# theteamatx/x-edr-trajectory-planning

Measured on AMD Instinct MI355X. Metric: time-optimal path timings/s (7-DOF, 2000 s-samples), 1/2/4/8 MI355X + %HBM roofline, higher is better.
Workload: dtype f64

## Files before the change

### x-edr-trajectory-planning_amd/csrc/tpamd_sweep_inst.hip

```cpp
#include "tpamd_launch.h"
#include "tpamd_sweep_joint.h"

#if !defined(TPAMD_INST_D) || !defined(TPAMD_INST_E)
#error "compile with -DTPAMD_INST_D=<joints> -DTPAMD_INST_E=<0|2>"
#endif

namespace tpamd {

template <>
void launch_sweep_joint<TPAMD_INST_D, TPAMD_INST_E>(int B, hipStream_t st, int N, int max_loops,
                                                    const JointSource &src, const Workspace &ws,
                                                    const tpamd_path_outputs *out) {
  hipLaunchKernelGGL((k_sweep_joint<TPAMD_INST_D, TPAMD_INST_E>), dim3(B), dim3(128),
                     (sweep_joint_lds_bytes<TPAMD_INST_D, TPAMD_INST_E>(N)), st, N, max_loops, src, ws,
                     out->time, out->s, out->sd, out->sdd, out->last_extremal_index,
                     out->max_time_increment, out->status, out->qd, out->qdd);
}

template <>
hipError_t configure_sweep_joint<TPAMD_INST_D, TPAMD_INST_E>() {
  return hipFuncSetAttribute(reinterpret_cast<const void *>(&k_sweep_joint<TPAMD_INST_D, TPAMD_INST_E>),
                             hipFuncAttributeMaxDynamicSharedMemorySize, 160 * 1024);
}

template <>
hipError_t sweep_joint_attributes<TPAMD_INST_D, TPAMD_INST_E>(hipFuncAttributes *attr) {
  return hipFuncGetAttributes(attr, reinterpret_cast<const void *>(&k_sweep_joint<TPAMD_INST_D, TPAMD_INST_E>));
}

}
```

### x-edr-trajectory-planning_amd/csrc/tpamd_sweep_joint.h

```cpp
#pragma once

#include <type_traits>

#include "tpamd_kernels.h"

namespace tpamd {

__device__ __forceinline__ double uniform_f64(double v) {
  const int lo = __builtin_amdgcn_readfirstlane(__double2loint(v));
  const int hi = __builtin_amdgcn_readfirstlane(__double2hiint(v));
  return __hiloint2double(hi, lo);
}
__device__ __forceinline__ double readlane_f64(double v, int lane) {
  const int lo = __builtin_amdgcn_readlane(__double2loint(v), lane);
  const int hi = __builtin_amdgcn_readlane(__double2hiint(v), lane);
  return __hiloint2double(hi, lo);
}
__device__ __forceinline__ int uniform_i32(int v) { return __builtin_amdgcn_readfirstlane(v); }
__device__ __forceinline__ int lds_word(const int *p) {
  return *(const volatile __attribute__((address_space(3))) int *)p;
}

template <int CTRL>
__device__ __forceinline__ double dpp_f64(double v) {
// ... 1160 lines not shown
        const bool iso_k = iso_at(at_l, N, k), iso_km1 = iso_at(at_l, N, k - 1),
                   iso_km2 = iso_at(at_l, N, k - 2);
        const bool l_mod = iso_k || iso_km2;
        const double m_l = l_mod ? z0[k - 1] : m0[k - 1];
        const double fsmax_l = l_mod ? Xz[k - 1] : X0[k - 1];
        const double m_c = iso_km1 ? z0[k] : m0[k];
        const double X_c = iso_km1 ? Xz[k] : X0[k];
        const double Y_c = iso_km1 ? Xz[k] : Y0[k];
        const double m_r = iso_k ? z0[k + 1] : m0[k + 1];
        const double Y_r = iso_k ? Xz[k + 1] : Y0[k + 1];
        const double fsmin_r = iso_k ? Yz[k + 1] : Y0[k + 1];
        const double sd2p = (m_r - m_c) / ds;
        const double sd2p_min = 2 * Y_c;
        const double sd2p_max = 2 * X_c;
        const bool sink_or_source = (sd2p < sd2p_min) || (sd2p > sd2p_max);
        const bool skipped_sdd = (X_c > 0) && (Y_r < 0);
        const bool skipped_sd2 = (m_c > m_l - kTiny) && (m_c > m_r - kTiny);
        if ((skipped_sd2 || skipped_sdd) && sink_or_source) {
          const double fw = m_l + 2.0 * ds * fsmax_l;
          const double bw = m_r - 2.0 * ds * fsmin_r;
          double mn = z0[k];
          if (fw < mn) mn = fw;
          if (bw < mn) mn = bw;
          ws.fix_val[pb + k] = (0.0 < mn) ? mn : 0.0;
          flag = 1;
        }
      }
      ff_l[k] = flag;
    };
    auto drain_detect = [&]() {
      JointSweep<D, E>::wave_lds_sync();
      for (int e0 = 0; e0 < nslow; e0 += 64)
        if (e0 + lane < nslow) detect_one(slow[e0 + lane]);
      nslow = 0;
      JointSweep<D, E>::wave_lds_sync();
    };
    double m0c[UF], X0c[UF], Y0c[UF];
    auto load_segment = [&](int cb) {
#pragma unroll
      for (int u = 0; u < UF; u++) {
        const int c = cb + 2 * u + w;
        const int k = 62 * c + lane - 1;
        const int kc = (c >= 1 && 62 * c + 62 < N) ? k : cl(k);
        m0c[u] = m0[kc]; X0c[u] = X0[kc]; Y0c[u] = Y0[kc];
      }
    };
    const bool owner = (lane >= 1) && (lane <= 62);
    for (int seg = 0; seg < nsg; seg++) {
    const int cb = seg * kSegChunks;
    load_segment(cb);
    unsigned listed = 0u;
#pragma unroll
    for (int u = 0; u < UF; u++) {
      const int k = 62 * (cb + 2 * u + w) + lane - 1;
      const bool inside = owner && (k >= 1) && (k <= N - 2);
      const int kb = max(k, 2);
      const bool near_iso = (iso_l[kb] | iso_l[kb - 1] | iso_l[kb - 2]) != 0;
      const double m_c = m0c[u], X_c = X0c[u], Y_c = Y0c[u];
      const double m0l = dpp_f64<0x138>(m_c);
      const double m0r = dpp_f64<0x130>(m_c), Y0r = dpp_f64<0x130>(Y_c);
      const double sd2p = (m0r - m_c) / ds;
      const double sd2p_min = 2 * Y_c;
      const double sd2p_max = 2 * X_c;
      const bool sink_or_source = (sd2p < sd2p_min) || (sd2p > sd2p_max);
      const bool skipped_sdd = (X_c > 0) && (Y0r < 0);
      const bool skipped_sd2 = (m_c > m0l - kTiny) && (m_c > m0r - kTiny);
      const bool fix = (skipped_sd2 || skipped_sdd) && sink_or_source;
      const bool to_list = inside && (near_iso || fix);
      if (owner && k >= 0 && k < N && !to_list) ff_l[k] = 0;
      listed |= (unsigned)to_list << u;
    }
    list_samples(listed, cb);
    drain_detect();
    }
    __threadfence_block();
    __syncthreads();
    TPAMD_ACCC(21, tp0);

    auto final_one = [&](int j, double &m, double &X, double &Y, double &m_next) -> bool {
      bool refit = false;
      m = 0.0; X = 0.0; Y = 0.0; m_next = 0.0;
      const bool f_next = (j + 1 <= N - 2) && ff_l[j + 1];
      const bool f_self = ff_l[j];
      const bool f_prev = (j >= 1) && ff_l[j - 1];
      const bool iso_p = iso_at(at_l, N, j - 1), iso_n = iso_at(at_l, N, j + 1);
      if (f_next || (!f_self && f_prev)) {
        m = z0[j];
        if (iso_p || iso_n) { X = Xz[j]; Y = Yz[j]; }
        else refit = true;
      } else if (f_self) {
        m = fv[j];
        refit = true;
      } else if (iso_n) {
        m = z0[j]; X = Xz[j]; Y = Yz[j];
      } else if (iso_p) {
        m = z0[j]; X = Xz[j]; Y = Xz[j];
      } else {
        m = m0[j]; X = X0[j]; Y = Y0[j];
      }
      const int jn = j + 1;
      if (jn <= N - 1) {
        if (jn + 1 <= N - 2 && ff_l[jn + 1]) m_next = z0[jn];
        else if (ff_l[jn]) m_next = fv[jn];
        else if (ff_l[jn - 1]) m_next = z0[jn];
        else if (iso_at(at_l, N, jn + 1) || iso_at(at_l, N, jn - 1)) m_next = z0[jn];
        else m_next = m0[jn];
      }
      return refit;
    };
    auto drain_final = [&]() {
      JointSweep<D, E>::wave_lds_sync();
      for (int e0 = 0; e0 < nslow; e0 += 64) {
        const bool valid = e0 + lane < nslow;
        double m = 0.0, X = 0.0, Y = 0.0, m_next = 0.0;
        bool refit = false;
        int j = 0;
        if (valid) {
          j = slow[e0 + lane];
          refit = final_one(j, m, X, Y, m_next);
          if (!refit) P.finalize(j, m, X, Y, m_next);
        }
        if (P.count + 64 > kRefitCap) P.template flush<true>(diag);
        P.append(refit, j, m, m_next);
      }
      nslow = 0;
      JointSweep<D, E>::wave_lds_sync();
    };
    for (int seg = 0; seg < nsg; seg++) {
    const int cb = seg * kSegChunks;
    if (!kOne) load_segment(cb);
    unsigned listed = 0u;
#pragma unroll
    for (int u = 0; u < UF; u++) {
      const int j = 62 * (cb + 2 * u + w) + lane - 1;
      const bool mine = owner && (j >= 0) && (j < N);
      const int jb = max(j, 1);
      const bool busy = (ff_l[jb - 1] | ff_l[jb] | ff_l[jb + 1] | ff_l[jb + 2] |
                         iso_l[jb - 1] | iso_l[jb] | iso_l[jb + 1] | iso_l[jb + 2]) != 0;
      const double m0r = dpp_f64<0x130>(m0c[u]);
      if (mine && !busy) P.finalize(j, m0c[u], X0c[u], Y0c[u], (j + 1 <= N - 1) ? m0r : 0.0);
      listed |= (unsigned)(mine && busy) << u;
    }
    list_samples(listed, cb);
    drain_final();
    }
    P.template flush<true>(diag);
    __threadfence_block();
    __syncthreads();
    TPAMD_ACCC(22, tp0);
    };
    if (nseg == 1) fast_form(std::true_type{});
    else fast_form(std::false_type{});
    return;
  }

  for (int base = 64 * w; base < N; base += 128) {
    const int j = base + lane;
    const bool need = (j < N) & ((iso_l[cl(j - 1)] | iso_l[cl(j + 1)]) != 0);
    if (P.count + 64 > kRefitCap) P.template flush<false>(diag);
    P.append(need, j, need ? z0[j] : 0.0, 0.0);
  }
  P.template flush<false>(diag);
  __threadfence_block();
  __syncthreads();
  TPAMD_ACCC(20, tp0);

  for (int k0 = tid; k0 < N; k0 += 128 * U) {
    double m0l[U], m0c[U], m0r[U], z0l[U], z0c[U], z0r[U], X0l[U], X0c[U], Y0c[U], Y0r[U];
    double Xzl[U], Xzc[U], Xzr[U], Yzr[U];
#pragma unroll
    for (int u = 0; u < U; u++) {
      const int k = k0 + 128 * u;
      const int kl = cl(k - 1), kc = cl(k), kr = cl(k + 1);
      m0l[u] = m0[kl]; m0c[u] = m0[kc]; m0r[u] = m0[kr];
      X0l[u] = X0[kl]; X0c[u] = X0[kc];
      Y0c[u] = Y0[kc]; Y0r[u] = Y0[kr];
      const bool ik = iso_at(at_l, N, k), ik1 = iso_at(at_l, N, k - 1), ik2 = iso_at(at_l, N, k - 2);
      z0l[u] = (ik || ik2) ? z0[kl] : 0.0;
      z0c[u] = ik1 ? z0[kc] : 0.0;
      z0r[u] = ik ? z0[kr] : 0.0;
      Xzl[u] = (ik || ik2) ? Xz[kl] : 0.0;
      Xzc[u] = ik1 ? Xz[kc] : 0.0;
      Xzr[u] = ik ? Xz[kr] : 0.0;
      Yzr[u] = ik ? Yz[kr] : 0.0;
    }
#pragma unroll
    for (int u = 0; u < U; u++) {
      const int k = k0 + 128 * u;
      if (k >= N) continue;
      uint8_t flag = 0;
      if (k >= 1 && k <= N - 2) {
        const bool iso_k = iso_at(at_l, N, k), iso_km1 = iso_at(at_l, N, k - 1),
                   iso_km2 = iso_at(at_l, N, k - 2);
        const bool l_mod = iso_k || iso_km2;
        const double m_l = l_mod ? z0l[u] : m0l[u];
        const double fsmax_l = l_mod ? Xzl[u] : X0l[u];
        const double m_c = iso_km1 ? z0c[u] : m0c[u];
        const double X_c = iso_km1 ? Xzc[u] : X0c[u];
        const double Y_c = iso_km1 ? Xzc[u] : Y0c[u];
        const double m_r = iso_k ? z0r[u] : m0r[u];
        const double Y_r = iso_k ? Xzr[u] : Y0r[u];
        const double fsmin_r = iso_k ? Yzr[u] : Y0r[u];
        const double sd2p = (m_r - m_c) / ds;
        const double sd2p_min = 2 * Y_c;
        const double sd2p_max = 2 * X_c;
        const bool sink_or_source = (sd2p < sd2p_min) || (sd2p > sd2p_max);
        const bool skipped_sdd = (X_c > 0) && (Y_r < 0);
        const bool skipped_sd2 = (m_c > m_l - kTiny) && (m_c > m_r - kTiny);
        if ((skipped_sd2 || skipped_sdd) && sink_or_source) {
          const double fw = m_l + 2.0 * ds * fsmax_l;
          const double bw = m_r - 2.0 * ds * fsmin_r;
          double mn = z0[k];
          if (fw < mn) mn = fw;
          if (bw < mn) mn = bw;
          ws.fix_val[pb + k] = (0.0 < mn) ? mn : 0.0;
          flag = 1;
        }
      }
      ff_l[k] = flag;
    }
  }
  __threadfence_block();
  __syncthreads();
  TPAMD_ACCC(21, tp0);

  for (int base = 256 * w; base < N; base += 512) {
    double m0c[U], z0c[U], X0c[U], Y0c[U], Xzc[U], Yzc[U], fvc[U], m0n[U], z0n[U], fvn[U];
#pragma unroll
    for (int u = 0; u < U; u++) {
      const int j = base + 64 * u + lane;
      const int jc = cl(j), jn = cl(j + 1);
      m0c[u] = m0[jc]; z0c[u] = z0[jc]; X0c[u] = X0[jc]; Y0c[u] = Y0[jc];
      m0n[u] = m0[jn]; z0n[u] = z0[jn];
      const bool near_iso = iso_at(at_l, N, jc - 1) || iso_at(at_l, N, jc + 1);
      Xzc[u] = near_iso ? Xz[jc] : 0.0;
      Yzc[u] = near_iso ? Yz[jc] : 0.0;
      fvc[u] = ff_l[jc] ? fv[jc] : 0.0;
      fvn[u] = ff_l[jn] ? fv[jn] : 0.0;
    }
#pragma unroll
    for (int u = 0; u < U; u++) {
      const int j = base + 64 * u + lane;
      const bool active = j < N;
      double m = 0.0, X = 0.0, Y = 0.0, m_next = 0.0;
      bool refit = false;
      if (active) {
        const bool f_next = (j + 1 <= N - 2) && ff_l[j + 1];
        const bool f_self = ff_l[j];
        const bool f_prev = (j >= 1) && ff_l[j - 1];
        const bool iso_p = iso_at(at_l, N, j - 1), iso_n = iso_at(at_l, N, j + 1);
        if (f_next || (!f_self && f_prev)) {
          m = z0c[u];
          if (iso_p || iso_n) { X = Xzc[u]; Y = Yzc[u]; }
          else refit = true;
        } else if (f_self) {
          m = fvc[u];
          refit = true;
        } else if (iso_n) {
          m = z0c[u]; X = Xzc[u]; Y = Yzc[u];
        } else if (iso_p) {
          m = z0c[u]; X = Xzc[u]; Y = Xzc[u];
        } else {
          m = m0c[u]; X = X0c[u]; Y = Y0c[u];
        }
        const int jn = j + 1;
        if (jn <= N - 1) {
          if (jn + 1 <= N - 2 && ff_l[jn + 1]) m_next = z0n[u];
          else if (ff_l[jn]) m_next = fvn[u];
          else if (ff_l[jn - 1]) m_next = z0n[u];
          else if (iso_at(at_l, N, jn + 1) || iso_at(at_l, N, jn - 1)) m_next = z0n[u];
          else m_next = m0n[u];
        }
        if (!refit) P.finalize(j, m, X, Y, m_next);
      }
      if (P.count + 64 > kRefitCap) P.template flush<true>(diag);
      P.append(refit, j, m, m_next);
    }
  }
  P.template flush<true>(diag);
  __threadfence_block();
  __syncthreads();
  TPAMD_ACCC(22, tp0);
}

template <int D, int E = 0>
struct SweepLds {
  static constexpr int R = 2 * D + E + 2;
  static constexpr int kRingDoubles = 2 * 2 * TileCfg<D>::kSamples * R;
  __host__ __device__ static constexpr int n2(int N) { return (N + 1) & ~1; }
  __host__ __device__ static constexpr int words(int N) { return ((N + 31) / 32 + 1) & ~1; }
  __host__ __device__ static constexpr int type_bytes(int N) { return ((N + 15) / 16) * 16; }
  __host__ __device__ static constexpr size_t bytes(int N) {
    return (size_t)n2(N) * 8 + (size_t)kRingDoubles * 8 + type_bytes(N) + 64 +
           2 * (size_t)words(N) * 4 + 16 * 8 + 32;
  }
};
template <int D, int E = 0>
__host__ __device__ inline size_t sweep_joint_lds_bytes(int N) {
  return SweepLds<D, E>::bytes(N);
}

constexpr int kSweepWavesPerEu = 2;
constexpr int kSweepWavesPerEuWide = 1;
template <int D, int E = 0>
__global__ void __launch_bounds__(128)
__attribute__((amdgpu_waves_per_eu((D > 8) ? kSweepWavesPerEuWide : kSweepWavesPerEu,
                                   (D > 8) ? kSweepWavesPerEuWide : kSweepWavesPerEu)))
k_sweep_joint(int stride, int max_loops, JointSource src, Workspace ws, double *t_out, double *s_out,
              double *sd_out, double *sdd_out, int32_t *lei_out, double *dtmax_out,
              int32_t *status_out, double *qd_out, double *qdd_out) {
  extern __shared__ double lds[];
  typedef JointSweep<D, E> JS;
  typedef SweepLds<D, E> LL;
  const int b = uniform_i32(path_of_block(ws, blockIdx.x));
  const int lane = threadIdx.x & 63;
  const int N = path_samples(ws, b, stride);
  const int w = uniform_i32((int)(threadIdx.x >> 6));
  const int tid = threadIdx.x;
  const size_t pb = (size_t)b * stride;
  const uint32_t bits = ws.err_bits[b];
  if (bits & kErrSkip) return;
  if (bits) {
    if (tid == 0) {
      status_out[b] = status_from_bits(bits);
      if (lei_out) lei_out[b] = 0;
      if (dtmax_out) dtmax_out[b] = -1.0;
    }
    return;
  }
  JS S;
  S.N = N; S.lane = lane;
  S.ds = ws.ds[b];
  S.two_ds = 2.0 * S.ds;
  S.sd2 = lds;
  double *ring = lds + LL::n2(N);
  S.tiles = ring + (size_t)w * 2 * JS::kTile * JS::R;
  uint8_t *typel = reinterpret_cast<uint8_t *>(ring + LL::kRingDoubles);
  S.typel = typel;
  int *xchg = reinterpret_cast<int *>(typel + LL::type_bytes(N));
  const int nw = LL::words(N);
  uint32_t *dirty = reinterpret_cast<uint32_t *>(xchg + 16);
  uint32_t *zero = dirty + nw;
  double *aml = reinterpret_cast<double *>(zero + nw);
  double *red = aml + 16;
  S.dirty = dirty;
  S.aml = aml;
  S.sdd_g = sdd_out + pb;
  S.m_g = ws.m + pb;
  S.rec = src.q12 + pb * JS::R;
  S.qd_g = qd_out ? qd_out + pb * D : nullptr;
  S.qdd_g = qdd_out ? qdd_out + pb * D : nullptr;
  S.end_idx = 0;
  S.tag0 = -1; S.tag1 = -1;
  double *sd2 = S.sd2;
  const double sd_start = ws.sd_start[b];
#ifdef TPAMD_DIAG
  long long(&diag)[32] = S.diag;
  long long(&diagx)[kDiagExt] = S.diagx;
  for (int k = 0; k < 32; k++) diag[k] = 0;
  for (int k = 0; k < kDiagExt; k++) diagx[k] = 0;
  volatile long long *fw_stamp = reinterpret_cast<volatile long long *>(red + 2);
#define TPAMD_DIAG_PTR S.diag
#else
#define TPAMD_DIAG_PTR nullptr
#endif
  boundary_passes_for_path<D, E>(src, ws, b, N, stride, tid, reinterpret_cast<uint8_t *>(sd2),
                           reinterpret_cast<uint8_t *>(sd2) + LL::type_bytes(N),
                           reinterpret_cast<char *>(ring), typel, (ws.keep_boundary & 1) != 0,
                           TPAMD_DIAG_PTR);
  constexpr int C = 2 * D + E;
  const double *lim_lo = src.lim + (size_t)b * 2 * C, *lim_hi = lim_lo + C;
  {
    typedef JointLayout<D> L;
    const double kInf = __longlong_as_double(0x7ff0000000000000LL);
    const bool is_cand = lane < L::kCandLanes;
    const int c = is_cand ? lane / L::PARTS : 0;
    const int p = lane % L::PARTS;
    const int r = c >> 1;
    S.own_off = r;
    S.lim = is_cand ? ((c & 1) ? lim_hi[r] : lim_lo[r]) : qnan();
#pragma unroll
    for (int k = 0; k < L::RPL; k++) {
      int j = p + k * L::PARTS;
      if (j >= D) j = (p < D) ? p : 0;
      S.chk_off[k] = j;
      S.chk_hi[k] = lim_hi[j];
    }
    const bool is_vel = lane < D;
    S.vel_off = is_vel ? lane : 0;
    S.vel_hi = is_vel ? lim_hi[D + lane] : kInf;
    S.vel_lo = is_vel ? 0.0 : -kInf;
    S.vel_mode = 0;
    if (E > 0) {
      if (lane >= D && lane < D + E) {
        S.vel_off = D;
        S.vel_mode = 1 + (lane - D);
        S.vel_hi = lim_hi[2 * D + (lane - D)];
        S.vel_lo = lim_lo[2 * D + (lane - D)];
      }
#pragma unroll
      for (int k = 0; k < (E ? E : 1); k++) S.ex_hi[k] = lim_hi[2 * D + k];
    }
  }
  S.row_lo = (lane < C) ? lim_lo[lane] : 0.0;
  S.row_hi = (lane < C) ? lim_hi[lane] : 0.0;
  {
    typedef JointLayout<D> L;
    const double kInf = __longlong_as_double(0x7ff0000000000000LL);
    const int p = lane & (L::GRP - 1);
#pragma unroll
    for (int i = 0; i < L::CPL; i++) {
      const int cand = p + L::GRP * i;
      const bool has = cand < 2 * D;
      const int row = has ? (cand >> 1) : 0;
      S.v_off[i] = row;
      S.v_lim[i] = has ? ((cand & 1) ? lim_hi[row] : lim_lo[row]) : qnan();
    }
#pragma unroll
    for (int i = 0; i < L::VPL; i++) {
      const int row = p + L::GRP * i;
      const bool has = row < D;
      S.vv_off[i] = has ? row : 0;
      S.vv_hi[i] = has ? lim_hi[D + row] : kInf;
      S.va_hi[i] = has ? lim_hi[row] : kInf;
    }
  }

  for (int i = tid; i < N; i += 128) {
    sd2[i] = qnan();
    S.sdd_g[i] = qnan();
  }
  for (int i = tid; i < 2 * nw; i += 128) dirty[i] = 0u;
  if (tid < D) aml[tid] = ws.amax ? ws.amax[(size_t)b * D + tid] : 0.0;
  __syncthreads();
  if (tid == 0) {
    xchg[2] = 0;
    xchg[6] = 0;
    sd2[0] = sd_start * sd_start;
    sd2[N - 1] = 0;
  }
  __syncthreads();

  int status = 0;
  int iforw_lo = 0, iback_hi = N - 1, iback_lo, iforw_hi, icrit, icrit_lo, icrit_hi;
  typename JS::Prefetch pf;
  pf.tag = -1;
  TPAMD_T0C(t_all);
  int emitted_hi = 0, upper_lo = N;
  bool first_pair_in_order = false;
  if (w == 0) {
    const int r = S.template add_extremal<false>(iback_hi, pf);
    if (lane == 0) { xchg[0] = r; xchg[7] = S.end_idx; }
  } else {
    const int r = S.template add_extremal<true>(iforw_lo, pf);
    if (lane == 0) { xchg[1] = r; xchg[8] = S.end_idx; }
  }
  __threadfence_block();
  __syncthreads();
  const int end_b = uniform_i32(xchg[7]), end_f = uniform_i32(xchg[8]);
  if (!(end_f + 70 < end_b)) {
    first_pair_in_order = true;
    for (int i = tid; i < N; i += 128) {
      sd2[i] = qnan();
      S.sdd_g[i] = qnan();
    }
    __syncthreads();
    if (tid == 0) {
      sd2[0] = sd_start * sd_start;
      sd2[N - 1] = 0;
    }
    __threadfence_block();
    __syncthreads();
  }
  if (first_pair_in_order) {
    if (w == 0) {
      const int r = S.template add_extremal<false>(iback_hi, pf);
      if (lane == 0) xchg[0] = r;
    }
    __threadfence_block();
    __syncthreads();
    if (w == 1) {
      const int r = S.template add_extremal<true>(iforw_lo, pf);
      if (lane == 0) xchg[1] = r;
    } else {
      upper_lo = min(S.end_idx + 3, N);
      S.emit_range(upper_lo, N - 1, 0, 1);
    }
    __threadfence_block();
    __syncthreads();
  }
  iback_lo = uniform_i32(xchg[0]);
  iforw_hi = uniform_i32(xchg[1]);
  TPAMD_ACCC(9, t_all);
  icrit_hi = iback_lo;
  if ((iforw_hi < icrit_hi) && ((icrit_hi < N - 2) && (icrit_hi >= 2))) {
    if (w == 0) S.put_sd2(icrit_hi, qnan());
    icrit_hi++;
    iback_lo++;
  }
  icrit_lo = iforw_hi;
  const int zlast = uniform_i32(S.last_flagged_below(icrit_hi));
  const double *m_g = ws.m + pb;
  if (max_loops <= 0) max_loops = max(100, 10 * N);
  double *crit_m = reinterpret_cast<double *>(xchg + 10);
  auto post_next_critical_point = [&](int lo) {
    TPAMD_T0(t0);
    int ic = uniform_i32(S.next_critical_point(lo, icrit_hi, zlast));
    TPAMD_ACC(2, t0);
#if defined(TPAMD_DIAG) && !defined(TPAMD_DIAG_LIGHT)
    {
      TPAMD_T0(tl_);
      if (ic != S.next_critical_point_literal(lo, icrit_hi)) TPAMD_CNT(7);
      TPAMD_ACC(18, tl_);
    }
#endif
    if (ic < 0 || ic >= N) ic = (int)(0.5 * (lo + icrit_hi));
    const double mc = m_g[min(max(ic, 0), N - 1)], mp = m_g[min(max(ic - 1, 0), N - 1)];
    if (ic >= 1) {
      const int ts = ic / JS::kTile;
      const int tag = (ts & 1) ? S.tag1 : S.tag0;
      if (tag != ts && pf.tag != ts) S.issue_tile_loads(ts, pf);
    }
    if (lane == 0) {
      xchg[9] = ic;
      crit_m[0] = mc;
      crit_m[1] = mp;
    }
  };
  __syncthreads();
  if (w == 1 && iforw_hi < icrit_hi) post_next_critical_point(icrit_lo);
  __threadfence_block();
  __syncthreads();
  for (int loop = 0; loop < max_loops; loop++) {
    if (iforw_hi >= icrit_hi) break;
    TPAMD_CNT(11);
#ifdef TPAMD_DIAG
    int bw_case = 2;
    long long bw_left = 0;
#endif
    icrit = uniform_i32(xchg[9]);
    const double m_c = uniform_f64(crit_m[0]), m_p = uniform_f64(crit_m[1]);
    if (w == 0 && icrit >= 1) {
      const int ts = (icrit - 1) / JS::kTile;
      const int tag = (ts & 1) ? S.tag1 : S.tag0;
      if (tag != ts && pf.tag != ts) S.issue_tile_loads(ts, pf);
    }
    if (icrit > 0 && icrit < N - 1 && w == 0) S.put_sd2(icrit, m_c);
    if (icrit < 1) { status = 10; break; }
    if (m_p <= m_c) {
      iback_hi = icrit - 1;
      if (w == 0) S.put_sd2(icrit - 1, m_p);
    } else {
      iback_hi = icrit;
    }
    iforw_lo = icrit;
    __syncthreads();
    {
      TPAMD_T0C(t0);
      if (w == 0) {
        const int r = S.template add_extremal<false>(iback_hi, pf, true);
        if (lane == 0) xchg[0] = r;
#ifdef TPAMD_DIAG
        const bool fw_was_done = lds_word(xchg + 6) == loop + 1;
#endif
        TPAMD_T0C(te);
        emitted_hi = uniform_i32(S.emit_range(max(min(S.end_idx - 1, emitted_hi), 0), icrit - 1,
                                              0, 1, xchg + 6, loop + 1));
        TPAMD_ACCC(12, te);
#ifdef TPAMD_DIAG
        bw_case = fw_was_done ? 0 : (lds_word(xchg + 6) == loop + 1) ? 1 : 2;
        bw_left = tpamd_stamp();
#endif
      } else {
        const int r = S.template add_extremal<true>(iforw_lo, pf, false, true);
#ifdef TPAMD_DIAG
        { const long long t = tpamd_stamp(); if (lane == 0) fw_stamp[0] = t; }
#endif
        if (lane == 0) {
          xchg[1] = r;
          *reinterpret_cast<volatile int *>(xchg + 6) = loop + 1;
        }
        if (r < icrit_hi) post_next_critical_point(r);
#ifdef TPAMD_DIAG
        { const long long t = tpamd_stamp(); if (lane == 0) fw_stamp[1] = t; }
#endif
      }
      TPAMD_ACCC(0, t0);
    }
    {
      TPAMD_T0C(t0);
      __threadfence_block();
#ifdef TPAMD_DIAG
      const long long fenced = tpamd_stamp();
#endif
      __syncthreads();
      TPAMD_ACCC(1, t0);
#ifdef TPAMD_DIAG
      if (w == 0) {
        const long long fw_done = fw_stamp[0], fw_at_c = fw_stamp[1];
        const long long fw_wait = (fenced > fw_at_c) ? fenced - fw_at_c : 0;
        diagx[0] += bw_case == 0;
        diagx[1] += bw_case == 1;
        diagx[2] += bw_case == 2;
        diagx[7] += fenced - t0;
        if (bw_case == 1) {
          diagx[3] += bw_left - fw_done;
          diagx[4] += fenced - t0;
          diagx[5] += fw_wait;
        } else if (bw_case == 0) {
          diagx[6] += fw_wait;
        }
      }
#endif
    }
    iback_lo = uniform_i32(xchg[0]);
    iforw_hi = uniform_i32(xchg[1]);
    if (iback_lo > icrit_lo) { status = 7; break; }
    icrit_lo = iforw_hi;
  }
  TPAMD_ACCC(5, t_all);
  if (lane == 0) {
    if (w == 0) { xchg[4] = emitted_hi; xchg[5] = upper_lo; }
    else xchg[3] = S.end_idx;
  }
  __threadfence_block();
  __syncthreads();

  TPAMD_T0C(t_tail);
  const double ds = S.ds;
  double *sdd = S.sdd_g;
  {
    int has_nan = 0;
    if (status == 0)
      for (int idx = tid; idx < N; idx += 128)
        if (isnan(sd2[idx])) has_nan = 1;
    if (has_nan) xchg[2] = 1;
    __syncthreads();
    if (status == 0 && xchg[2] != 0) status = 8;
  }
  if (status == 0) {
    for (int base = 0; base < N; base += 512) {
      double cur[4];
#pragma unroll
      for (int u = 0; u < 4; u++) cur[u] = sdd[min(base + 128 * u + tid, N - 1)];
#pragma unroll
      for (int u = 0; u < 4; u++) {
        const int idx = base + 128 * u + tid;
        if (idx < N && isnan(cur[u])) {
          const auto r = src.at(b, stride, idx);
          const double s2 = sd2[idx];
          const bool has_next = idx < N - 1, has_prev = idx > 0;
          double res = 0.0;
          bool done = false;
          if (has_next && has_prev) {
            const double c = 0.25 / ds * (sd2[idx + 1] - sd2[idx - 1]);
            if (rows_valid(r, C, c, s2)) { res = c; done = true; }
          }
          if (!done && has_next) {
            const double c = 0.5 / ds * (sd2[idx + 1] - s2);
            if (rows_valid(r, C, c, s2)) { res = c; done = true; }
          }
          if (!done && has_prev) {
            const double c = 0.5 / ds * (s2 - sd2[idx - 1]);
            if (rows_valid(r, C, c, s2)) { res = c; done = true; }
          }
          sdd[idx] = res;
          atomicOr(&dirty[idx >> 5], 1u << (idx & 31));
        }
      }
    }
    if (w == 0) {
      const double sdd_start = ws.sdd_start[b];
      const auto r0 = src.at(b, stride, 0);
      const double s20 = sd2[0];
      bool bad = false;
      for (int i = lane; i < C; i += 64) {
        const double v = r0.a(i) * sdd_start + r0.b(i) * s20;
        if (v + kTiny < r0.lo(i) || v - kTiny > r0.hi(i)) bad = true;
      }
      if (!__any(bad) && lane == 0) {
        sdd[0] = sdd_start;
        atomicOr(&dirty[0], 1u);
      }
    }
    if (sd2[N - 1] != 0) status = 9;
  }
  if (status != 0) {
    if (tid == 0) {
      status_out[b] = status;
      if (lei_out) lei_out[b] = 0;
      if (dtmax_out) dtmax_out[b] = -1.0;
    }
#ifdef TPAMD_DIAG
    if (lane == 0 && ws.diag)
      for (int k = 0; k < 32; k++) ws.diag[(size_t)b * kDiagRow + 32 * w + k] = S.diag[k];
#endif
    return;
  }
  __threadfence_block();
  __syncthreads();
  {
    const int e_hi = uniform_i32(xchg[4]), u_lo = uniform_i32(xchg[5]);
    const int f_end = uniform_i32(xchg[3]);
    S.emit_range(e_hi, min(max(u_lo - 1, f_end + 1), N - 1), w, 2);
  }
  TPAMD_ACC(13, t_tail);
  const double t0v = ws.t_start[b];
  const double s0 = ws.s_start[b], s1 = ws.s_end[b];
  double *tl = ring;
  constexpr int kCap = LL::kRingDoubles;
  double tprev = t0v;
  double dtmax = 0.0;
  for (int base = 0; base < N; base += kCap) {
    const int n = min(kCap, N - base);
    const bool last_chunk = base + kCap >= N;
    TPAMD_T0(t_a);
    for (int k = tid; k < n; k += 128) {
      const int idx = base + k;
      const double s2 = sd2[idx];
      const double sdv = sqrt(s2);
      double dt = 0.0;
      if (idx >= 1) {
        const double s2p = sd2[idx - 1];
        if ((s2p > 0) || (s2 > 0)) {
          dt = 2.0 * ds / (sqrt(s2p) + sdv);
        } else {
          const uint32_t m0 = 1u << ((idx - 1) & 31), m1 = 1u << (idx & 31);
          atomicOr(&zero[(idx - 1) >> 5], m0); atomicOr(&dirty[(idx - 1) >> 5], m0);
          atomicOr(&zero[idx >> 5], m1);       atomicOr(&dirty[idx >> 5], m1);
        }
      }
      tl[k] = dt;
      sd_out[pb + idx] = sdv;
      s_out[pb + idx] = (idx == N - 1) ? s1 : ds * idx + s0;
      ws.sd2[pb + idx] = s2;
      if (ws.sd2_out) ws.sd2_out[pb + idx] = s2;
      if (dt > dtmax) dtmax = dt;
    }
    __syncthreads();
    TPAMD_ACC(16, t_a);
    TPAMD_T0(t_b);
    if (w == 0) {
      double t = tprev;
      OrderedSumMasks osm;
      osm.init(lane);
      for (int k0 = 0; k0 < n; k0 += 64) {
        const int k = k0 + lane;
        const double dtv = (k < n) ? tl[k] : 0.0;
        const bool finite = __ballot(!(dtv <= DBL_MAX)) == 0ull;
        const double y = finite ? ordered_sum64_finite(t, dtv, osm) : ordered_sum64(t, dtv);
        if (k < n) tl[k] = y;
        t = readlane_f64(y, 63);
      }
      JS::wave_lds_sync();
      tprev = t;
    } else {
      if (base == 0) {
        int lei = 0;
        const int start = (1 > N - 2) ? 1 : N - 2;
        bool found = false;
        for (int top = start; top >= 1 && !found; top -= 256) {
          double a[4], mm[4];
#pragma unroll
          for (int u = 0; u < 4; u++) {
            const int ic = max(top - 64 * u - lane, 0);
            a[u] = sdd[ic];
            mm[u] = m_g[ic];
          }
#pragma unroll
          for (int u = 0; u < 4; u++) {
            const int idx = top - 64 * u - lane;
            const bool hit = (idx >= 1) & ((a[u] > 0.0) | (fabs(sd2[max(idx, 0)] - mm[u]) < kTiny));
            const unsigned long long mask = __ballot(hit);
            if (mask && !found) { lei = top - 64 * u - (__ffsll((long long)mask) - 1); found = true; }
          }
        }
        if (lane == 0 && lei_out) lei_out[b] = lei;
      }
      if (last_chunk) {
        for (int wi = lane; wi < nw; wi += 64) {
          uint32_t zb = zero[wi];
          while (zb) {
            const int i = __ffs((int)zb) - 1;
            sdd[wi * 32 + i] = 0.0;
            zb &= zb - 1u;
          }
        }
        __threadfence_block();
        if (S.emitting()) {
          int *list = reinterpret_cast<int *>(typel);
          const int list_cap = LL::type_bytes(N) / 4;
          int count = 0;
          bool all = false;
          for (int wb = 0; wb < nw; wb += 64) {
            const int wi = wb + lane;
            uint32_t db = (wi < nw) ? dirty[wi] : 0u;
            const int c = __popc(db);
            int incl = c;
#pragma unroll
            for (int off = 1; off < 64; off <<= 1) {
              const int o = __shfl_up(incl, off, 64);
              if (lane >= off) incl += o;
            }
            const int total = count + __shfl(incl, 63, 64);
            if (total > list_cap) { all = true; break; }
            int pos = count + incl - c;
            while (db) {
              const int i = __ffs((int)db) - 1;
              list[pos++] = wi * 32 + i;
              db &= db - 1u;
            }
            count = total;
          }
          JS::wave_lds_sync();
          constexpr int PER = 64 / D;
          constexpr int U = 4;
          const int g = lane / D, d = lane - g * D;
          const f64x2 *rec2 = reinterpret_cast<const f64x2 *>(S.rec);
          const int total = all ? N : count;
          for (int k0 = 0; k0 < total; k0 += PER * U) {
            f64x2 pr[U];
            double s2v[U], av[U];
            int id[U];
            bool ok[U];
#pragma unroll
            for (int u = 0; u < U; u++) {
              const int k = k0 + u * PER + g;
              ok[u] = (g < PER) && (k < total);
              const int kk = ok[u] ? k : k0;
              id[u] = all ? kk : list[kk];
              pr[u] = rec2[(size_t)id[u] * (JS::R / 2) + d];
              s2v[u] = sd2[id[u]];
              av[u] = sdd[id[u]];
            }
#pragma unroll
            for (int u = 0; u < U; u++)
              if (ok[u]) S.emit_value(id[u], d, pr[u], sqrt(s2v[u]), av[u], aml[d]);
          }
        }
      }
    }
    TPAMD_ACC(17, t_b);
    __syncthreads();
    for (int k = tid; k < n; k += 128) t_out[pb + base + k] = tl[k];
    if (!last_chunk) __syncthreads();
  }
  dtmax = wave_max_f64(dtmax);
  if (lane == 0) red[w] = dtmax;
  __syncthreads();
  if (tid == 0) {
    status_out[b] = 0;
    if (dtmax_out) dtmax_out[b] = (red[0] > red[1]) ? red[0] : red[1];
  }
  TPAMD_ACCC(3, t_tail);
  TPAMD_ACCC(15, t_all);
#ifdef TPAMD_DIAG
  if (lane == 0 && ws.diag) {
    for (int k = 0; k < 32; k++) ws.diag[(size_t)b * kDiagRow + 32 * w + k] = S.diag[k];
    for (int k = 0; k < kDiagExt; k++) ws.diag[(size_t)b * kDiagRow + 64 + kDiagExt * w + k] = S.diagx[k];
  }
#endif
}

static __global__ void __launch_bounds__(64)
k_rebuild_time(int N, int paths_per_shard, size_t shard_stride, const double *sd_base,
               const double *ds_base, const double *t_start_base, const int32_t *ns, double *t_out) {
  const int p = blockIdx.x, lane = threadIdx.x;
  const int r = p / paths_per_shard, b = p - r * paths_per_shard;
  const double *sd = sd_base + (size_t)r * shard_stride + (size_t)b * N;
  const double ds = ds_base[(size_t)r * shard_stride + b];
  double t = t_start_base[(size_t)r * shard_stride + b];
  double *out = t_out + (size_t)p * N;
  const int Nb = ns ? min(ns[p], N) : N;
  OrderedSumMasks osm;
  osm.init(lane);
  for (int k0 = 0; k0 < Nb; k0 += 64) {
    const int i = k0 + lane;
    const bool in = i < Nb;
    const double sdv = in ? sd[i] : 0.0;
    const double sdp = (in && i >= 1) ? sd[i - 1] : 0.0;
    double dt = 0.0;
    if (in && i >= 1 && ((sdp > 0) || (sdv > 0))) dt = 2.0 * ds / (sdp + sdv);
    const bool finite = __ballot(!(dt <= DBL_MAX)) == 0ull;
    const double y = finite ? ordered_sum64_finite(t, dt, osm) : ordered_sum64(t, dt);
    if (in) out[i] = y;
    t = readlane_f64(y, 63);
  }
}

}
```

Measured before the change: 2.167 million.

## Reload sweep kernel args from kernarg segment to cut SGPR live ranges

Packs the sweep kernel's arguments into one struct. The kernel reads fields directly from the kernarg segment pointer near where they are used instead of holding them live across the whole kernel. Tail-phase pointers and LDS offsets are recomputed after the main loop behind asm barriers, and the row validity check becomes a branch-free unrolled loop over C constraints. The aim is to relieve scalar register pressure and spills in the long-lived kernel. The cost is extra scalar loads and address recomputation.

```diff
diff --git a/x-edr-trajectory-planning_amd/csrc/tpamd_sweep_inst.hip b/x-edr-trajectory-planning_amd/csrc/tpamd_sweep_inst.hip
--- a/x-edr-trajectory-planning_amd/csrc/tpamd_sweep_inst.hip
+++ b/x-edr-trajectory-planning_amd/csrc/tpamd_sweep_inst.hip
@@ -11,10 +11,10 @@
 void launch_sweep_joint<TPAMD_INST_D, TPAMD_INST_E>(int B, hipStream_t st, int N, int max_loops,
                                                     const JointSource &src, const Workspace &ws,
                                                     const tpamd_path_outputs *out) {
+  const SweepArgs args = {N, max_loops, src, ws, out->time, out->s, out->sd, out->sdd,
+                          out->last_extremal_index, out->max_time_increment, out->status, out->qd, out->qdd};
   hipLaunchKernelGGL((k_sweep_joint<TPAMD_INST_D, TPAMD_INST_E>), dim3(B), dim3(128),
-                     (sweep_joint_lds_bytes<TPAMD_INST_D, TPAMD_INST_E>(N)), st, N, max_loops, src, ws,
-                     out->time, out->s, out->sd, out->sdd, out->last_extremal_index,
-                     out->max_time_increment, out->status, out->qd, out->qdd);
+                     (sweep_joint_lds_bytes<TPAMD_INST_D, TPAMD_INST_E>(N)), st, args);
 }
 
 template <>
diff --git a/x-edr-trajectory-planning_amd/csrc/tpamd_sweep_joint.h b/x-edr-trajectory-planning_amd/csrc/tpamd_sweep_joint.h
--- a/x-edr-trajectory-planning_amd/csrc/tpamd_sweep_joint.h
+++ b/x-edr-trajectory-planning_amd/csrc/tpamd_sweep_joint.h
@@ -1486,16 +1486,53 @@
 
 constexpr int kSweepWavesPerEu = 2;
 constexpr int kSweepWavesPerEuWide = 1;
+
+struct SweepArgs {
+  int stride, max_loops;
+  JointSource src;
+  Workspace ws;
+  double *t_out, *s_out, *sd_out, *sdd_out;
+  int32_t *lei_out;
+  double *dtmax_out;
+  int32_t *status_out;
+  double *qd_out, *qdd_out;
+};
+typedef const __attribute__((address_space(4))) SweepArgs *SweepArgsPtr;
+__device__ __forceinline__ SweepArgsPtr sweep_args() {
+  SweepArgsPtr p = (SweepArgsPtr)__builtin_amdgcn_kernarg_segment_ptr();
+  asm volatile("" : "+s"(p));
+  return p;
+}
+template <typename T>
+__device__ __forceinline__ T sweep_arg_copy(const __attribute__((address_space(4))) T *p) {
+  T v;
+  __builtin_memcpy(&v, p, sizeof(T));
+  return v;
+}
+
+template <int C, class R>
+__device__ __forceinline__ bool rows_valid_all(const R &r, double sdd, double sd2) {
+  bool bad = false;
+#pragma unroll
+  for (int i = 0; i < C; i++) {
+    const double v = r.a(i) * sdd + r.b(i) * sd2;
+    bad = bad | (v + kTiny < r.lo(i)) | (v - kTiny > r.hi(i));
+  }
+  return !bad;
+}
+
 template <int D, int E = 0>
 __global__ void __launch_bounds__(128)
 __attribute__((amdgpu_waves_per_eu((D > 8) ? kSweepWavesPerEuWide : kSweepWavesPerEu,
                                    (D > 8) ? kSweepWavesPerEuWide : kSweepWavesPerEu)))
-k_sweep_joint(int stride, int max_loops, JointSource src, Workspace ws, double *t_out, double *s_out,
-              double *sd_out, double *sdd_out, int32_t *lei_out, double *dtmax_out,
-              int32_t *status_out, double *qd_out, double *qdd_out) {
+k_sweep_joint(SweepArgs) {
   extern __shared__ double lds[];
   typedef JointSweep<D, E> JS;
   typedef SweepLds<D, E> LL;
+  const SweepArgsPtr args = sweep_args();
+  const int stride = args->stride;
+  const JointSource src = sweep_arg_copy(&args->src);
+  const Workspace ws = sweep_arg_copy(&args->ws);
   const int b = uniform_i32(path_of_block(ws, blockIdx.x));
   const int lane = threadIdx.x & 63;
   const int N = path_samples(ws, b, stride);
@@ -1506,12 +1543,13 @@
   if (bits & kErrSkip) return;
   if (bits) {
     if (tid == 0) {
-      status_out[b] = status_from_bits(bits);
-      if (lei_out) lei_out[b] = 0;
-      if (dtmax_out) dtmax_out[b] = -1.0;
+      args->status_out[b] = status_from_bits(bits);
+      if (args->lei_out) args->lei_out[b] = 0;
+      if (args->dtmax_out) args->dtmax_out[b] = -1.0;
     }
     return;
   }
+  double *const sdd_out = args->sdd_out, *const qd_out = args->qd_out, *const qdd_out = args->qdd_out;
   JS S;
   S.N = N; S.lane = lane;
   S.ds = ws.ds[b];
@@ -1650,7 +1688,8 @@
     }
     __syncthreads();
     if (tid == 0) {
-      sd2[0] = sd_start * sd_start;
+      const double sd_again = sweep_args()->ws.sd_start[b];
+      sd2[0] = sd_again * sd_again;
       sd2[N - 1] = 0;
     }
     __threadfence_block();
@@ -1684,7 +1723,8 @@
   }
   icrit_lo = iforw_hi;
   const int zlast = uniform_i32(S.last_flagged_below(icrit_hi));
-  const double *m_g = ws.m + pb;
+  const double *m_g = S.m_g;
+  int max_loops = sweep_args()->max_loops;
   if (max_loops <= 0) max_loops = max(100, 10 * N);
   double *crit_m = reinterpret_cast<double *>(xchg + 10);
   auto post_next_critical_point = [&](int lo) {
@@ -1811,6 +1851,19 @@
   __syncthreads();
 
   TPAMD_T0C(t_tail);
+  const SweepArgsPtr targs = sweep_args();
+  int n_t = N;
+  asm volatile("" : "+s"(n_t));
+  double *const ring_t = lds + LL::n2(n_t);
+  uint8_t *const typel_t = reinterpret_cast<uint8_t *>(ring_t + LL::kRingDoubles);
+  int *const xchg_t = reinterpret_cast<int *>(typel_t + LL::type_bytes(n_t));
+  const int nw_t = LL::words(n_t);
+  uint32_t *const dirty_t = reinterpret_cast<uint32_t *>(xchg_t + 16);
+  uint32_t *const zero_t = dirty_t + nw_t;
+  double *const aml_t = reinterpret_cast<double *>(zero_t + nw_t);
+  double *const red_t = aml_t + 16;
+  const int stride_t = targs->stride;
+  const size_t pb_t = (size_t)b * stride_t;
   const double ds = S.ds;
   double *sdd = S.sdd_g;
   {
@@ -1818,9 +1871,9 @@
     if (status == 0)
       for (int idx = tid; idx < N; idx += 128)
         if (isnan(sd2[idx])) has_nan = 1;
-    if (has_nan) xchg[2] = 1;
+    if (has_nan) xchg_t[2] = 1;
     __syncthreads();
-    if (status == 0 && xchg[2] != 0) status = 8;
+    if (status == 0 && xchg_t[2] != 0) status = 8;
   }
   if (status == 0) {
     for (int base = 0; base < N; base += 512) {
@@ -1831,31 +1884,31 @@
       for (int u = 0; u < 4; u++) {
         const int idx = base + 128 * u + tid;
         if (idx < N && isnan(cur[u])) {
-          const auto r = src.at(b, stride, idx);
+          const auto r = sweep_arg_copy(&targs->src).at(b, stride_t, idx);
           const double s2 = sd2[idx];
           const bool has_next = idx < N - 1, has_prev = idx > 0;
           double res = 0.0;
           bool done = false;
           if (has_next && has_prev) {
             const double c = 0.25 / ds * (sd2[idx + 1] - sd2[idx - 1]);
-            if (rows_valid(r, C, c, s2)) { res = c; done = true; }
+            if (rows_valid_all<C>(r, c, s2)) { res = c; done = true; }
           }
           if (!done && has_next) {
             const double c = 0.5 / ds * (sd2[idx + 1] - s2);
-            if (rows_valid(r, C, c, s2)) { res = c; done = true; }
+            if (rows_valid_all<C>(r, c, s2)) { res = c; done = true; }
           }
           if (!done && has_prev) {
             const double c = 0.5 / ds * (s2 - sd2[idx - 1]);
-            if (rows_valid(r, C, c, s2)) { res = c; done = true; }
+            if (rows_valid_all<C>(r, c, s2)) { res = c; done = true; }
           }
           sdd[idx] = res;
-          atomicOr(&dirty[idx >> 5], 1u << (idx & 31));
+          atomicOr(&dirty_t[idx >> 5], 1u << (idx & 31));
         }
       }
     }
     if (w == 0) {
-      const double sdd_start = ws.sdd_start[b];
-      const auto r0 = src.at(b, stride, 0);
+      const double sdd_start = targs->ws.sdd_start[b];
+      const auto r0 = sweep_arg_copy(&targs->src).at(b, stride_t, 0);
       const double s20 = sd2[0];
       bool bad = false;
       for (int i = lane; i < C; i += 64) {
@@ -1864,34 +1917,36 @@
       }
       if (!__any(bad) && lane == 0) {
         sdd[0] = sdd_start;
-        atomicOr(&dirty[0], 1u);
+        atomicOr(&dirty_t[0], 1u);
       }
     }
     if (sd2[N - 1] != 0) status = 9;
   }
   if (status != 0) {
     if (tid == 0) {
-      status_out[b] = status;
-      if (lei_out) lei_out[b] = 0;
-      if (dtmax_out) dtmax_out[b] = -1.0;
+      targs->status_out[b] = status;
+      if (targs->lei_out) targs->lei_out[b] = 0;
+      if (targs->dtmax_out) targs->dtmax_out[b] = -1.0;
     }
 #ifdef TPAMD_DIAG
-    if (lane == 0 && ws.diag)
-      for (int k = 0; k < 32; k++) ws.diag[(size_t)b * kDiagRow + 32 * w + k] = S.diag[k];
+    if (long long *const dg = targs->ws.diag; lane == 0 && dg)
+      for (int k = 0; k < 32; k++) dg[(size_t)b * kDiagRow + 32 * w + k] = S.diag[k];
 #endif
     return;
   }
   __threadfence_block();
   __syncthreads();
   {
-    const int e_hi = uniform_i32(xchg[4]), u_lo = uniform_i32(xchg[5]);
-    const int f_end = uniform_i32(xchg[3]);
+    const int e_hi = uniform_i32(xchg_t[4]), u_lo = uniform_i32(xchg_t[5]);
+    const int f_end = uniform_i32(xchg_t[3]);
     S.emit_range(e_hi, min(max(u_lo - 1, f_end + 1), N - 1), w, 2);
   }
   TPAMD_ACC(13, t_tail);
-  const double t0v = ws.t_start[b];
-  const double s0 = ws.s_start[b], s1 = ws.s_end[b];
-  double *tl = ring;
+  const double t0v = targs->ws.t_start[b];
+  const double s0 = targs->ws.s_start[b], s1 = targs->ws.s_end[b];
+  double *const t_out = targs->t_out, *const s_out = targs->s_out, *const sd_out = targs->sd_out;
+  double *const sd2_ws = targs->ws.sd2, *const sd2_out = targs->ws.sd2_out;
+  double *tl = ring_t;
   constexpr int kCap = LL::kRingDoubles;
   double tprev = t0v;
   double dtmax = 0.0;
@@ -1910,15 +1965,15 @@
           dt = 2.0 * ds / (sqrt(s2p) + sdv);
         } else {
           const uint32_t m0 = 1u << ((idx - 1) & 31), m1 = 1u << (idx & 31);
-          atomicOr(&zero[(idx - 1) >> 5], m0); atomicOr(&dirty[(idx - 1) >> 5], m0);
-          atomicOr(&zero[idx >> 5], m1);       atomicOr(&dirty[idx >> 5], m1);
+          atomicOr(&zero_t[(idx - 1) >> 5], m0); atomicOr(&dirty_t[(idx - 1) >> 5], m0);
+          atomicOr(&zero_t[idx >> 5], m1);       atomicOr(&dirty_t[idx >> 5], m1);
         }
       }
       tl[k] = dt;
-      sd_out[pb + idx] = sdv;
-      s_out[pb + idx] = (idx == N - 1) ? s1 : ds * idx + s0;
-      ws.sd2[pb + idx] = s2;
-      if (ws.sd2_out) ws.sd2_out[pb + idx] = s2;
+      sd_out[pb_t + idx] = sdv;
+      s_out[pb_t + idx] = (idx == N - 1) ? s1 : ds * idx + s0;
+      sd2_ws[pb_t + idx] = s2;
+      if (sd2_out) sd2_out[pb_t + idx] = s2;
       if (dt > dtmax) dtmax = dt;
     }
     __syncthreads();
@@ -1959,11 +2014,11 @@
             if (mask && !found) { lei = top - 64 * u - (__ffsll((long long)mask) - 1); found = true; }
           }
         }
-        if (lane == 0 && lei_out) lei_out[b] = lei;
+        if (int32_t *const lei_out = targs->lei_out; lane == 0 && lei_out) lei_out[b] = lei;
       }
       if (last_chunk) {
-        for (int wi = lane; wi < nw; wi += 64) {
-          uint32_t zb = zero[wi];
+        for (int wi = lane; wi < nw_t; wi += 64) {
+          uint32_t zb = zero_t[wi];
           while (zb) {
             const int i = __ffs((int)zb) - 1;
             sdd[wi * 32 + i] = 0.0;
@@ -1972,13 +2027,13 @@
         }
         __threadfence_block();
         if (S.emitting()) {
-          int *list = reinterpret_cast<int *>(typel);
+          int *list = reinterpret_cast<int *>(typel_t);
           const int list_cap = LL::type_bytes(N) / 4;
           int count = 0;
           bool all = false;
-          for (int wb = 0; wb < nw; wb += 64) {
+          for (int wb = 0; wb < nw_t; wb += 64) {
             const int wi = wb + lane;
-            uint32_t db = (wi < nw) ? dirty[wi] : 0u;
+            uint32_t db = (wi < nw_t) ? dirty_t[wi] : 0u;
             const int c = __popc(db);
             int incl = c;
 #pragma unroll
@@ -2019,29 +2074,29 @@
             }
 #pragma unroll
             for (int u = 0; u < U; u++)
-              if (ok[u]) S.emit_value(id[u], d, pr[u], sqrt(s2v[u]), av[u], aml[d]);
+              if (ok[u]) S.emit_value(id[u], d, pr[u], sqrt(s2v[u]), av[u], aml_t[d]);
           }
         }
       }
     }
     TPAMD_ACC(17, t_b);
     __syncthreads();
-    for (int k = tid; k < n; k += 128) t_out[pb + base + k] = tl[k];
+    for (int k = tid; k < n; k += 128) t_out[pb_t + base + k] = tl[k];
     if (!last_chunk) __syncthreads();
   }
   dtmax = wave_max_f64(dtmax);
-  if (lane == 0) red[w] = dtmax;
+  if (lane == 0) red_t[w] = dtmax;
   __syncthreads();
   if (tid == 0) {
-    status_out[b] = 0;
-    if (dtmax_out) dtmax_out[b] = (red[0] > red[1]) ? red[0] : red[1];
+    targs->status_out[b] = 0;
+    if (double *const dtmax_out = targs->dtmax_out) dtmax_out[b] = (red_t[0] > red_t[1]) ? red_t[0] : red_t[1];
   }
   TPAMD_ACCC(3, t_tail);
   TPAMD_ACCC(15, t_all);
 #ifdef TPAMD_DIAG
-  if (lane == 0 && ws.diag) {
-    for (int k = 0; k < 32; k++) ws.diag[(size_t)b * kDiagRow + 32 * w + k] = S.diag[k];
-    for (int k = 0; k < kDiagExt; k++) ws.diag[(size_t)b * kDiagRow + 64 + kDiagExt * w + k] = S.diagx[k];
+  if (long long *const dg = targs->ws.diag; lane == 0 && dg) {
+    for (int k = 0; k < 32; k++) dg[(size_t)b * kDiagRow + 32 * w + k] = S.diag[k];
+    for (int k = 0; k < kDiagExt; k++) dg[(size_t)b * kDiagRow + 64 + kDiagExt * w + k] = S.diagx[k];
   }
 #endif
 }
```

Result: no change. 2.184 million (median of 6 runs) (+0.8%).
